# a-ludi/dentist

Measured on AMD Instinct MI355X. Metric: gap-bases closed/sec, higher is better.
Workload: dtype u8

## Files before the change

### dentist_amd/_lib.py

```python
import ctypes
import os
import weakref

import numpy as np

_HERE = os.path.dirname(os.path.abspath(__file__))


def lib_path():
    return os.environ.get("DH_DEV_LIB") or os.path.join(_HERE, "libdentist_hip.so")


class DhError(RuntimeError):
    def __init__(self, code, msg):
        super().__init__(f"libdentist_hip error {code}: {msg}")
        self.code = code


class AlignOpts(ctypes.Structure):
    _fields_ = [(n, ctypes.c_int32) for n in (
        "k", "hmin", "band_shift", "tspace", "min_len", "pen", "xdrop", "max_err_ppm", "max_cand",
        "max_la", "tcap", "strands", "skip_self", "dmax", "width", "kmer_mod", "algo")]


# ... 34 lines not shown
    "contig_left", "status", "nreads", "ref_read", "ref_read_id", "crop_left", "crop_right", "left_aepos",
    "right_abpos", "ins_begin", "ins_end", "comp", "cons_len", "left_diffs", "right_diffs", "join")]
    + [("cons_off", "<i8"), ("contig_right", "<i4"), ("pad", "<i4")])

EXACT_HIT_DTYPE = np.dtype([("query", "<i4"), ("ref", "<i4"), ("begin", "<i8"), ("end", "<i8"), ("complement", "<i4"),
                            ("pad", "<i4")])

LA_DTYPE = np.dtype([("tlen", "<i4"), ("diffs", "<i4"), ("abpos", "<i4"), ("bbpos", "<i4"),
                     ("aepos", "<i4"), ("bepos", "<i4"), ("flags", "<u4"), ("aread", "<i4"),
                     ("bread", "<i4"), ("pad", "<i4"), ("toff", "<i8")])

SYMBOLS = [
    "dh_last_error", "dh_abi_version", "dh_ctx_create", "dh_ctx_destroy", "dh_ctx_sync",
    "dh_default_align_opts", "dh_db_create", "dh_db_destroy", "dh_db_drop_cache", "dh_db_nreads",
    "dh_db_total_bases", "dh_la_set_destroy", "dh_la_set_count", "dh_la_set_trace_len",
    "dh_la_set_records", "dh_la_set_trace", "dh_la_set_tspace", "dh_get_align_stats", "dh_get_cum_stats", "dh_get_mjoin_counts", "dh_get_join_counts", "dh_get_tjoin_counts", "dh_join_hit_capacity",
    "dh_ctx_release_scratch",
    "dh_align_db",
    "dh_las_write", "dh_las_read", "dh_default_process_opts", "dh_collect_spanning", "dh_pileups_destroy",
    "dh_pileups_count", "dh_pileups_get", "dh_process_pileups", "dh_insertions_destroy",
    "dh_insertions_count", "dh_insertions_records", "dh_insertions_bases", "dh_insertions_bases_len",
    "dh_get_process_stats", "dh_dazz_create_dam", "dh_dazz_create_db", "dh_dazz_split", "dh_dazz_open",
    "dh_dazz_close", "dh_dazz_nreads", "dh_dazz_first_id", "dh_dazz_bases", "dh_dazz_offsets",
    "dh_dazz_origin", "dh_dazz_fpulse", "dh_dazz_header", "dh_dazz_read_mask", "dh_dazz_write_mask",
    "dh_db_set_mask", "dh_output_fasta", "dh_tile_qv", "dh_consensus", "dh_las_merge",
    "dh_collect_candidates", "dh_pileups_create", "dh_pileups_select", "dh_align_db_block", "dh_la_set_merge",
    "dh_crop_pileups", "dh_cropped_create", "dh_cropped_destroy", "dh_cropped_npiles", "dh_cropped_records",
    "dh_cropped_nreads", "dh_cropped_pile", "dh_cropped_entry", "dh_cropped_read_id", "dh_cropped_offsets",
    "dh_cropped_bases", "dh_process_cropped", "dh_translate_trace_point", "dh_db_dust", "dh_db_get_mask",
    "dh_dazz_write_track", "dh_dazz_read_track", "dh_dazz_remove", "dh_dazz_flags",
    "dh_pileupdb_write", "dh_pileupdb_read", "dh_insertiondb_write", "dh_insertiondb_read", "dh_insertiondb_merge", "dh_chaindb_destroy",
# ... 312 lines not shown
        _check(lib().dh_get_mjoin_counts(self._h, out, int(reset)))
        return int(out[0]), int(out[1])

    def join_counts(self, reset=False):
        out = (ctypes.c_int64 * 4)()
        lib().dh_get_join_counts.argtypes = [ctypes.c_void_p, ctypes.c_void_p, ctypes.c_int32]
        _check(lib().dh_get_join_counts(self._h, out, int(reset)))
        return tuple(int(x) for x in out)

    def tjoin_counts(self, reset=False):
        out = (ctypes.c_int64 * 4)()
        lib().dh_get_tjoin_counts.argtypes = [ctypes.c_void_p, ctypes.c_void_p, ctypes.c_int32]
        _check(lib().dh_get_tjoin_counts(self._h, out, int(reset)))
        return tuple(int(x) for x in out)

    def cum_stats(self, reset=False):
        st = CumStats()
        _check(lib().dh_get_cum_stats(self._h, ctypes.byref(st), int(reset)))
        return st

    def remap_skipping_reads(self, contigs, reads, contig_ids, read_ids, opts, allowance):
        ci = np.ascontiguousarray(contig_ids, dtype=np.int32)
        ri = np.ascontiguousarray(read_ids, dtype=np.int32)
        h = ctypes.c_void_p()
        L = lib()
        L.dh_remap_skipping_reads.argtypes = [ctypes.c_void_p, ctypes.c_void_p, ctypes.c_void_p, ctypes.c_void_p, ctypes.c_int32,
                                              ctypes.c_void_p, ctypes.c_int32, ctypes.c_void_p, ctypes.c_int32,
                                              ctypes.POINTER(ctypes.c_void_p)]
        _check(L.dh_remap_skipping_reads(self._h, contigs._h, reads._h, ci.ctypes.data, len(ci), ri.ctypes.data, len(ri),
                                         ctypes.byref(opts), int(allowance), ctypes.byref(h)))
# ... 1618 lines not shown
```

### dentist_amd/csrc/dh_align.cpp

```cpp
#include <chrono>
#include <cmath>
#include <cstdio>
#include <cstdlib>
#include <cstring>
#include <numeric>
#include <functional>
#include <memory>
#include <mutex>
#include <thread>

#include "dh_internal.h"
#include "dh_join.h"
#include "dh_mjoin.h"
#include "dh_tjoin.h"
#include "dh_tile.h"
#include "dh_parallel.h"

#define fail dh_fail

#ifdef DH_SEED_PROF
extern "C" void dhk_seed_prof_dump();
extern "C" void dhk_join_prof_dump();
extern "C" void dhk_tile_prof_dump();
#endif
// ... 831 lines not shown
        tj_chunk = true;
    }
    const bool jn = r.use_join || mj_chunk || tj_chunk;
    const JoinView &jvx = mj_chunk ? jv_mj : (tj_chunk ? jv_tj : r.jv);
    const int tier_max = getenv("DH_SEED_NO16K") ? 8192 : 16384;
    const double kmers_per_read = (double)(B->h_off[(size_t)((item0 + ni) >> 1)] - B->h_off[(size_t)(item0 >> 1)]) /
                                  std::max(1, ni / 2) / std::max(1, o.kmer_mod);
    const double mean_hits = tj_chunk ? (double)tj_hits / std::max(1, ni / 2) : kmers_per_read * (2.0 * r.dens + 0.075);
    const bool wave_tier = (mj_chunk || tj_chunk) && ctx->seed_wave_tier && 1.5 * mean_hits <= 512.0 && !getenv("DH_SEED_NO_WAVE_TIER");
    int capj = std::min(std::max(r.cap, 2048), tier_max);
    if (mj_chunk || tj_chunk) {
        capj = 2048;
        while (capj < tier_max && 1.5 * mean_hits > capj) capj *= 2;
        if (wave_tier) capj = 512;
    }
    if (jn && capj > 4096) SCR(SLOT_FSCR, d_fscr, (size_t)ctx->ncu * DH_SEED_FSCR_BLOCKS_PER_CU * (capj > 8192 ? DH_SEED_FSCR_WORDS16 : DH_SEED_FSCR_WORDS))
    if (jn)
        dhk_seed_join(st, capj, r.bv, r.iv, r.dopt, jvx, (int32_t)item0, ni, c.candbase, c.ncandbase, c.nhitsbase, r.d_status,
                      r.d_queue + 1, ctx->ncu, d_fscr, nullptr, 0);
    else
        dhk_seed(st, r.cap, r.bv, r.iv, r.dopt, (int32_t)item0, ni, c.candbase, c.ncandbase, c.nhitsbase, r.d_status,
                 r.d_queue + 1, ctx->ncu, d_fscr);
    HIPCHK(hipGetLastError());
    int32_t status = 0;
    unsigned long long sm[4] = {0, 0, 0, 0};
    dhk_seed_summary(st, r.d_ncand, r.d_nhits, ni, r.d_summary);
    HIPCHK(hipMemcpyAsync(&status, r.d_status, sizeof(int32_t), hipMemcpyDeviceToHost, st));
    HIPCHK(hipMemcpyAsync(sm, r.d_summary, sizeof(sm), hipMemcpyDeviceToHost, st));
    HIPCHK(hipStreamSynchronize(st));
    if (mj_chunk && (status & DH_ST_MJ_POOL) && !(status & DH_ST_MJ_OVERFLOW) && !getenv("DH_MJOIN_PAGES")) {
        unsigned long long cnt2[2] = {0, 0};
        HIPCHK(hipMemcpyAsync(cnt2, r.d_mjctr_last + 10, sizeof(cnt2), hipMemcpyDeviceToHost, st));
        status &= ~DH_ST_MJ_POOL;
        HIPCHK(hipMemcpyAsync(r.d_status, &status, sizeof(int32_t), hipMemcpyHostToDevice, st));
// ... 36 lines not shown
            fprintf(stderr, "[seeds] %zu of %d reads overflow the wavefront-per-read tier: not used by this context any more\n", big.size(), ni / 2);
    }
    size_t redo_all = (size_t)ni / 50 + 8;
    if (r.cap >= 8192) redo_all = (size_t)ni / 4;
    if (const char *e = getenv("DH_SEED_BIG_PCT")) redo_all = (size_t)((double)ni * atof(e) / 200.0);
    if (getenv("DH_TRACE") && !big.empty())
        fprintf(stderr, "[seeds] cap %d: %zu of %d reads overflow (whole chunk again above %zu)\n", r.cap, big.size(), ni / 2, redo_all);
    if (!jn && big.size() > redo_all && r.cap < 16384) {
        r.cap *= 2;
        *redo = true;
        return DH_OK;
    }
    if (mj_chunk) ctx->mj_chunks++;
    if (tj_chunk) ctx->tj_last_hits += (int64_t)tj_hits;
    r.mj_skip_chunk = false;
    if (jn && capj < tier_max && !big.empty()) {
        std::vector<int32_t> huge;
        int32_t gcap2 = 0;
        for (int tier = capj < 2048 ? 2048 : 8192; tier <= tier_max; tier = tier < 8192 ? 8192 : tier * 2) {
            if (tier <= capj) continue;
            std::vector<int32_t> mid;
            huge.clear();
            gcap2 = 0;
            for (int32_t rd : big) {
                const size_t it = (size_t)(2 * (int64_t)rd - item0);
                const int32_t nh = r.h_nhits[it] + r.h_nhits[it + 1];
                if (nh <= tier)
                    mid.push_back(rd);
                else {
                    huge.push_back(rd);
                    gcap2 = std::max(gcap2, nh);
                }
            }
            if (!mid.empty()) {
                int32_t *d_mid;
                uint64_t *d_fscr2;
                SCR(SLOT_MID_LIST, d_mid, mid.size())
                SCR(SLOT_FSCR, d_fscr2, (size_t)ctx->ncu * DH_SEED_FSCR_BLOCKS_PER_CU * (tier > 8192 ? DH_SEED_FSCR_WORDS16 : DH_SEED_FSCR_WORDS))
                HIPCHK(hipMemcpyAsync(d_mid, mid.data(), sizeof(int32_t) * mid.size(), hipMemcpyHostToDevice, st));
                HIPCHK(hipMemsetAsync(r.d_queue + 1, 0, sizeof(uint32_t), st));
                dhk_seed_join(st, tier, r.bv, r.iv, r.dopt, jvx, (int32_t)item0, ni, c.candbase, c.ncandbase, c.nhitsbase, r.d_status,
                              r.d_queue + 1, ctx->ncu, d_fscr2, d_mid, (int32_t)mid.size());
                HIPCHK(hipGetLastError());
                HIPCHK(hipStreamSynchronize(st));
            }
            if (getenv("DH_TRACE"))
                fprintf(stderr, "[seeds] join tiers: %zu reads redone with %d entries, %zu left\n", mid.size(), tier, huge.size());
            big = huge;
        }
        gcap = gcap2;
    }
    if (!big.empty()) {
        if (gcap > (1 << 22)) return fail(DH_EOVERFLOW, "seed filter: more than 4M k-mer hits for one sequence; lower -t");
        int32_t pow2 = 1;
        while (pow2 < gcap) pow2 <<= 1;
        const size_t slab_words = 2 * (size_t)pow2 + ((size_t)pow2 + 1) / 2;
        const size_t per_launch = std::max<size_t>(1, (size_t)(2ull << 30) / (slab_words * 8));
// ... 495 lines not shown
```

### dentist_amd/csrc/dh_api.cpp

```cpp
#include <cstring>

#include "dh_internal.h"

static_assert(sizeof(dh_align_opts) == sizeof(DhOpts), "opts layout");
static_assert(sizeof(dh_la) == sizeof(DhLa), "la layout");
static_assert(sizeof(dh_la) == 48, "la size");

static thread_local std::string g_err;

int dh_fail(int code, const std::string &msg)
{
    g_err = msg;
    return code;
}
#define fail dh_fail

extern "C" const char *dh_last_error(void) { return g_err.c_str(); }
extern "C" int32_t dh_abi_version(void) { return 4; }



extern "C" int dh_ctx_create(int32_t device, void *stream, dh_ctx **out)
{
    if (!out) return fail(DH_EINVAL, "dh_ctx_create: out is NULL");
// ... 115 lines not shown
    if (reset) c->mj_chunks = c->mj_fallbacks = 0;
    return DH_OK;
}

extern "C" int dh_get_tjoin_counts(dh_ctx *c, int64_t *out4, int32_t reset)
{
    if (!c || !out4) return fail(DH_EINVAL, "dh_get_tjoin_counts: NULL");
    out4[0] = c->tj_calls;
    out4[1] = c->tj_fallbacks;
    out4[2] = c->tj_last_hits;
    out4[3] = c->tj_reruns;
    if (reset) c->tj_calls = c->tj_fallbacks = c->tj_last_hits = c->tj_reruns = 0;
    return DH_OK;
}

extern "C" int dh_get_join_counts(dh_ctx *c, int64_t *out4, int32_t reset)
{
    if (!c || !out4) return fail(DH_EINVAL, "dh_get_join_counts: NULL");
    out4[0] = c->join_launches;
    out4[1] = c->join_reruns;
    out4[2] = c->join_last_hits;
    out4[3] = c->join_first_cap;
    if (reset) c->join_launches = c->join_reruns = c->join_last_hits = c->join_first_cap = 0;
    return DH_OK;
}

extern "C" int dh_get_align_stats(dh_ctx *c, dh_align_stats *out)
{
    if (!c || !out) return fail(DH_EINVAL, "dh_get_align_stats: NULL");
    *out = c->stats;
// ... 32 lines not shown
```

### dentist_amd/csrc/dh_batch.cpp

```cpp
#include <atomic>
#include <cstdlib>
#include <cstring>
#include <exception>
#include <string>
#include <thread>

#include "dh_process.h"
#include "dh_parallel.h"

using namespace dhp;

extern "C" {
void dhk_gather_ranges16(hipStream_t st, const uint16_t *src, const int64_t *desc, int32_t n, uint16_t *dst);
}

namespace {

int select_trace_ranges(const dh_db *reads, const dh_la_set *set, const dh_pileups *piles, std::vector<int64_t> &desc, int64_t &total)
{
    const int64_t n = (int64_t)set->la.size();
    std::vector<uint8_t> need((size_t)reads->n, 0);
    for (const auto &t : piles->triples)
        for (size_t x = 0; x + 2 < t.size(); x += 3) {
            if (t[x] < 0 || t[x] >= reads->n) return dh_fail(DH_EINVAL, "dh_process_pileups_set: read id out of range");
// ... 200 lines not shown
        a.ms_index += b.ms_index; a.ms_seed += b.ms_seed; a.ms_wave += b.ms_wave; a.ms_gather += b.ms_gather;
        a.wave_launches += b.wave_launches; a.wave_cells += b.wave_cells; a.alignments += b.alignments; a.las += b.las;
        a.aligned_bp += b.aligned_bp; a.trace_values += b.trace_values; a.hits += b.hits; a.b_bases += b.b_bases;
        b = dh_cum_stats();
        dh_ctx *sc = ctx->sub[k - 1];
        ctx->join_launches += sc->join_launches;
        ctx->join_reruns += sc->join_reruns;
        ctx->join_last_hits += sc->join_last_hits;
        ctx->join_first_cap += sc->join_first_cap;
        sc->join_launches = sc->join_reruns = sc->join_last_hits = sc->join_first_cap = 0;
        ctx->tj_calls += sc->tj_calls;
        ctx->tj_fallbacks += sc->tj_fallbacks;
        ctx->tj_last_hits += sc->tj_last_hits;
        ctx->tj_reruns += sc->tj_reruns;
        sc->tj_calls = sc->tj_fallbacks = sc->tj_last_hits = sc->tj_reruns = 0;
    }
}

void fold_part_stats(const std::vector<PartOut> &po)
{
    ProcStats &ps = dh_proc_stats();
    for (size_t k = 1; k < po.size(); k++) {
        for (int i = 0; i < 7; i++) ps.ms[i] = std::max(ps.ms[i], po[k].st.ms[i]);
        for (int i = 0; i < 3; i++) ps.counters[i] += po[k].st.counters[i];
        for (int i = 0; i < 4; i++) ps.work[i] += po[k].st.work[i];
    }
}

dh_insertions *append_insertions(std::vector<PartOut> &po)
{
// ... 56 lines not shown
```

### dentist_amd/csrc/dh_internal.h

```cpp
#ifndef DH_INTERNAL_H
#define DH_INTERNAL_H

#include "../../include/dentist_hip.h"

#include <hip/hip_runtime.h>

#include <algorithm>
#include <string>
#include <new>
#include <utility>
#include <vector>

#include "dh_device.h"

#define DB_PAD 64
#define PK_PAD 128

hipError_t dh_dev_alloc(void **p, size_t bytes);
void dh_dev_free(void *p);
void dh_dev_trim();
template <typename T>
inline hipError_t dh_dev_alloc(T **p, size_t bytes)
{
    return dh_dev_alloc((void **)p, bytes);
// ... 79 lines not shown

#define DH_TJ_HIT_RATE0 0.14

struct dh_ctx {
    int device = 0;
    hipStream_t stream = nullptr;
    bool own_stream = false;
    int ncu = 0;
    hipEvent_t ev[8] = {};
    hipStream_t cstream = nullptr;
    hipEvent_t cev[4] = {};
    dh_align_stats stats = {};
    dh_cum_stats cum = {};
    double mj_hit_frac = 0.2;
    int seed_wave_tier = 1;
    int64_t mj_chunks = 0, mj_fallbacks = 0;
    int64_t tj_calls = 0, tj_fallbacks = 0, tj_last_hits = 0, tj_reruns = 0;
    double tj_hit_rate = DH_TJ_HIT_RATE0;
    double join_hit_rate = DH_JOIN_HIT_RATE0;
    int64_t join_launches = 0, join_reruns = 0, join_last_hits = 0, join_first_cap = 0;
    int32_t near_best_ppm = -1;
    dh_ctx *sub[3] = {nullptr, nullptr, nullptr};
    struct Arena {
        void *p = nullptr;
        size_t cap = 0;
    } arena[DH_SLOT_COUNT];
};
int dh_scratch(dh_ctx *ctx, DhSlot id, size_t bytes, void **out);
int dh_db_set_pflags(struct dh_db *db, const uint8_t *flags);

// ... 180 lines not shown
```

### dentist_amd/csrc/dh_join.h

```cpp
#ifndef DH_JOIN_H
#define DH_JOIN_H
#include <stdint.h>

#include "dh_device.h"

#define JP_THREADS 512
#define JP_PER 16
#define JP_POS (JP_THREADS * JP_PER)
#define JOIN_MAX_READS 512
#define JOIN_MAX_LEN (1 << 21)
#define JOIN_MAX_SLICES 512
#define JOIN_CAP 4096
#define JOIN_FILL 2300
#define JOIN_THREADS 512

#define DH_ST_JOIN_OVERFLOW 0x8
#define DH_ST_JOIN_HITCAP 0x10

struct JoinView {
    const int32_t *gfirst;
    const int32_t *gns;
    const int32_t *pfirst;
    const int2 *pblk;
    const int64_t *psubrow;
// ... 6 lines not shown
    unsigned long long *cursor;
    int64_t hits_cap;
    int32_t *status;
    int32_t npart, njoin;
    int32_t ns_fixed, read0;
};

#ifdef __cplusplus
extern "C" {
#endif
void dhk_join_part(hipStream_t st, JoinView jv, DbView B, int32_t k, int32_t kmer_mod);
void dhk_join(hipStream_t st, JoinView jv, DbView B, DhOpts o, const int64_t *goff, int32_t sepv);
void dhk_join_hist(hipStream_t st, JoinView jv, const int32_t *group, int32_t nreads, unsigned int *out4);
void dhk_seed_join(hipStream_t st, int cap, DbView B, IndexView ix, DhOpts o, JoinView jv, int32_t item0, int32_t nitems,
                   DhCand *cand, int32_t *ncand, int32_t *nhits, int32_t *status, uint32_t *queue, int32_t ncu,
                   uint64_t *fscr, const int32_t *read_list, int32_t nlist);
void dhk_seed_big_join(hipStream_t st, DbView B, IndexView ix, DhOpts o, JoinView jv, const int32_t *read_list,
                       int32_t nreads, uint64_t *gbuf, int32_t gcap, DhCand *cand, int32_t *ncand, int32_t *nhits,
                       int32_t *status, uint32_t *queue, int32_t ncu);
#ifdef __cplusplus
}
#endif
#endif
```

### dentist_amd/csrc/dh_seed.hip

```cpp
#include <hip/hip_runtime.h>
#include <type_traits>
#include <algorithm>
#include <cstdlib>
#include <stdio.h>
#include <stdint.h>
#include <stdlib.h>

#include "dh_device.h"
#include "dh_join.h"

#define LANES 64

#include "dh_kmer.h"


__device__ int g_seed_sort_refine = 1;
#define HIT_QBITS 24
#define HIT_QMASK ((1u << HIT_QBITS) - 1u)
#define SEED_THREADS 512
#define SEED_LOOKUP_THREADS 512
#define SEED_CCAP 256

__device__ __forceinline__ int64_t hitD(uint64_t h) { return (int64_t)(h >> HIT_QBITS); }
__device__ __forceinline__ int32_t hitQ(uint64_t h) { return (int32_t)(h & HIT_QMASK); }

__device__ __forceinline__ int32_t hit_cov(const uint64_t *h, int32_t i, int32_t k)
{
    if (i > 0 && hitD(h[i - 1]) == hitD(h[i])) {
        const int32_t dq = hitQ(h[i]) - hitQ(h[i - 1]);
        return dq < k ? dq : k;
    }
    return k;
}

#ifdef DH_SEED_PROF
__device__ unsigned long long g_seed_prof[12];
#define SP(i) if (tid == 0) { const unsigned long long t_ = wall_clock64(); atomicAdd(&g_seed_prof[i], t_ - tp_); tp_ = t_; }
#else
#define SP(i)
#endif
#define HIT_DBITS 39
template <int LCAP, bool JOIN, int NT, int CC>
__device__ void seed_item(const DbView &B, const IndexView &ix, const JoinView &jv,
                          const DhOpts &o, int32_t read0, int32_t work, int32_t slab,
                          DhCand *__restrict__ cand_out, int32_t *__restrict__ ncand_out,
                          int32_t *__restrict__ nhits_out, int32_t *__restrict__ status,
                          uint64_t *__restrict__ gbuf, int32_t gcap, const int32_t *__restrict__ read_list)
{
    __shared__ uint64_t lhits[LCAP > 0 ? LCAP : 1];
    __shared__ DhCand cands[2 * CC];
    __shared__ int64_t cband[2 * CC];
    __shared__ int32_t s_n, s_nc;

    const int32_t r = read_list ? read_list[work] : read0 + work;
    const int32_t item = 2 * r;
    uint64_t *hits = LCAP > 0 ? lhits : gbuf + (int64_t)slab * (2 * (int64_t)gcap + (gcap + 1) / 2);
    const int32_t CAP = LCAP > 0 ? LCAP : gcap;
    const int tid = threadIdx.x;
#ifdef DH_SEED_PROF
    unsigned long long tp_ = wall_clock64();
#endif
    if (tid == 0) {
        s_n = 0;
        s_nc = 0;
    }
    __syncthreads();
    const int64_t bo = B.off[r];
    const int32_t blen = (int32_t)(B.off[r + 1] - bo);
    const uint8_t *b = B.bases + bo;
    const uint64_t grp = B.group ? (uint64_t)B.group[r] : 0ull;
    const int k = o.k;
    const uint64_t mask = (1ull << (2 * k)) - 1;
    const int32_t npos = blen - k + 1;
    constexpr uint64_t ORI = 1ull << 63, PAL = 1ull << 62;

    if (JOIN) {
        uint64_t *segb = (uint64_t *)cands;
        uint32_t *sego = (uint32_t *)(cands + CC) + 1;
        __shared__ uint32_t s_jw[NT / LANES];
        const int32_t ns = jv.gns ? jv.gns[B.group[r]] : jv.ns_fixed;
        const int64_t srow = jv.gns ? jv.segrow[r] : (int64_t)(r - jv.read0) * jv.ns_fixed;
        uint32_t c = 0;
        if (tid < ns) {
            const uint64_t sg = jv.segtab[srow + tid];
            c = (uint32_t)(sg & 0xFFFFFFull);
            segb[tid] = sg >> 24;
        }
        uint32_t incl = c;
        for (int off = 1; off < LANES; off <<= 1) {
            const uint32_t up = __shfl_up(incl, off, LANES);
            if ((tid & (LANES - 1)) >= off) incl += up;
        }
        if ((tid & (LANES - 1)) == LANES - 1) s_jw[tid / LANES] = incl;
// ... 182 lines not shown
    if (n > CAP) {
        if (tid == 0) {
            if (LCAP == 0) atomicOr(status, DH_ST_HIT_OVERFLOW);
            ncand_out[item] = ncand_out[item + 1] = LCAP > 0 ? -1 : 0;
            nhits_out[item] = n;
            nhits_out[item + 1] = 0;
        }
        return;
    }
    if (n == 0) {
        if (tid == 0) ncand_out[item] = ncand_out[item + 1] = nhits_out[item] = nhits_out[item + 1] = 0;
        return;
    }
    int32_t N = 1;
    while (N < n) N <<= 1;
    constexpr bool SMALL = NT < SEED_THREADS;
    if (SMALL) {
        constexpr int E8 = LCAP / NT > 0 ? LCAP / NT : 1;
        uint64_t ky[E8];
        int32_t rk8[E8];
#pragma unroll
        for (int u = 0; u < E8; u++) {
            const int32_t i = tid + u * NT;
            ky[u] = i < n ? hits[i] : ~0ull;
            rk8[u] = 0;
        }
#define DH_RANK_KEYS(M_)                                                   \
    for (int32_t x = 0; x < n; x++) {                                      \
        const uint64_t h = hits[x];                                        \
        _Pragma("unroll") for (int u = 0; u < (M_ < E8 ? M_ : E8); u++) rk8[u] += h < ky[u] ? 1 : 0; \
    }
        if (n <= 2 * NT) {
// ... 15 lines not shown
        if (tid < n) {
            key = hits[tid];
#pragma unroll 4
            for (int32_t x = 0; x < n; x++) rk += hits[x] < key ? 1 : 0;
        }
        __syncthreads();
        if (tid < n)
            hits[rk] = key;
        else if (tid < N)
            hits[tid] = ~0ull;
        N = 1;
    } else if (LCAP == 0 || ((LCAP <= 8192 || JOIN) && (JOIN || LCAP >= 4096))) {
        constexpr int E = LCAP >= NT ? LCAP / NT : 1;
        constexpr int NB = 2048, NBH = NB / 2, SORT_BMAX = LCAP == 0 ? 384 : 256;
        constexpr uint64_t DM = (1ull << HIT_DBITS) - 1;
        static_assert(SMALL || sizeof(cands) >= NB * sizeof(uint32_t), "bucket counters overlay the candidate array");
        uint32_t *bcnt = (uint32_t *)cands;
        __shared__ unsigned long long s_dmin, s_dmax;
        __shared__ uint32_t s_bw[NT / LANES];
        __shared__ uint32_t s_bmax;
        constexpr int HV = 8, NB2 = 1024;
        constexpr bool REFINE = LCAP > 0 && !SMALL;
        static_assert(!REFINE || sizeof(cband) >= NB2 * sizeof(uint32_t), "the second pass's counters overlay the band array");
        uint32_t *fcnt = (uint32_t *)cband;
        __shared__ uint32_t s_nheavy, s_heavy[HV];
        for (int32_t i = tid; i < NB; i += NT) bcnt[i] = 0;
        if (tid == 0) {
            s_dmin = ~0ull;
            s_dmax = 0ull;
            s_bmax = 0;
            s_nheavy = 0;
        }
        unsigned long long dmin = ~0ull, dmax = 0ull;
        for (int32_t i = tid; i < n; i += NT) {
            const unsigned long long d = (hits[i] >> HIT_QBITS) & DM;
            dmin = d < dmin ? d : dmin;
            dmax = d > dmax ? d : dmax;
        }
        for (int off = LANES / 2; off > 0; off >>= 1) {
// ... 222 lines not shown
                    if (REFINE)
                        for (uint32_t hv = 0; hv < nheavy; hv++) heavy = heavy || s_heavy[hv] == bk;
                    if (heavy)
                        dst[u] = (uint32_t)i;
                    else
                        dst[u] = b0 + count_below(b0, b1, key, sh <= 32 - HIT_QBITS);
                }
            }
            __syncthreads();
#pragma unroll
            for (int u = 0; u < E; u++)
                if (tid + u * NT < n) hits[dst[u]] = ke[u];
            N = 1;
        } else {
#ifdef DH_SEED_PROF
            if (tid == 0) atomicAdd(&g_seed_prof[10], 1ull);
#endif
            for (int32_t i = n + tid; i < N; i += NT) hits[i] = ~0ull;
        }
    } else {
        for (int32_t i = n + tid; i < N; i += NT) hits[i] = ~0ull;
    }
    __syncthreads();
    for (int32_t kk = 2; kk <= N; kk <<= 1) {
        for (int32_t j = kk >> 1; j > 0; j >>= 1) {
            const bool cross = j >= 128;
            if (cross) __syncthreads();
            constexpr int SORT_U = (LCAP == 0 || LCAP >= 4096) ? 8 : 4;
            for (int32_t p0 = tid; p0 < (N >> 1); p0 += NT * SORT_U) {
                uint64_t xs[SORT_U], ys[SORT_U];
#pragma unroll
// ... 27 lines not shown
    __syncthreads();
    if (tid == 0) {
        int32_t lo = 0, hi = n;
        while (lo < hi) {
            const int32_t mid = (lo + hi) >> 1;
            if (hits[mid] >> 63)
                hi = mid;
            else
                lo = mid + 1;
        }
        nhits_out[item] = lo;
        nhits_out[item + 1] = n - lo;
    }
    SP(1)
    constexpr bool FASTB = LCAP <= 8192 || (JOIN && LCAP == 16384);
    constexpr bool FB_LDS = LCAP > 0 && LCAP <= 4096;
    constexpr bool FB_BIG = LCAP == 0;
    constexpr bool FB_WIDE = LCAP == 0 || LCAP == 16384;
    using bsum_t = typename std::conditional<FB_WIDE, uint64_t, uint32_t>::type;
    using bhead_t = typename std::conditional<FB_WIDE, uint32_t, uint16_t>::type;
    constexpr int HSH = FB_WIDE ? 32 : 18;
    constexpr bsum_t CMASK = ((bsum_t)1 << HSH) - 1;
    __shared__ uint32_t bsum_l[FB_LDS ? LCAP : 1];
    __shared__ uint16_t bhead_l[FB_LDS ? LCAP : 1];
    bsum_t *bsum = FB_LDS ? (bsum_t *)bsum_l
                          : (FB_BIG ? (bsum_t *)(hits + gcap) : (bsum_t *)(gbuf + (int64_t)slab * gcap));
    bhead_t *bhead = FB_LDS ? (bhead_t *)bhead_l : (bhead_t *)(bsum + (LCAP > 0 ? LCAP : gcap));
    __shared__ bsum_t s_wsum[NT / LANES];
    __shared__ int32_t s_nbig;
    constexpr int NBIG = NT < SEED_THREADS ? 8 : ((LCAP > 0 && LCAP <= 4096) ? 128 : 64);
    __shared__ int32_t bigc[NBIG][4];
    __shared__ unsigned long long s_bestkeys[NBIG];
    const int bs = o.band_shift;
    auto emit_cand = [&](int32_t slot, int32_t best_first, int32_t P, int64_t band) {
        const int64_t D = hitD(hits[best_first]) & ((1ll << HIT_DBITS) - 1);
        const int32_t q = hitQ(hits[best_first]);
        const int64_t gv = D - ix.sepv + q;
        const int32_t lo = ix.page_seq[gv >> 12];
        cands[slot].score = P;
        cands[slot].aseq = lo;
        cands[slot].apos = (int32_t)(gv - ix.goff[lo]);
        cands[slot].bpos = q;
        cband[slot] = band;
    };
    auto serial_seed = [&](int32_t i, int32_t e1) {
// ... 70 lines not shown
            if (slot >= 2 * CC) continue;
            if (e1 - i > 16) {
                const int32_t bslot = atomicAdd(&s_nbig, 1);
                if (bslot < NBIG) {
                    bigc[bslot][0] = i;
                    bigc[bslot][1] = e1;
                    bigc[bslot][2] = P;
                    bigc[bslot][3] = slot;
                    continue;
                }
            }
            emit_cand(slot, serial_seed(i, e1), P, band);
        }
        __syncthreads();
        SP(8)
        constexpr int GW = 16;
        const int32_t nbig = min(s_nbig, NBIG);
        const int gl = tid & (GW - 1);
        for (int32_t bc = tid / GW; bc < nbig; bc += NT / GW) {
            const int32_t i = bigc[bc][0], e1 = bigc[bc][1];
            unsigned long long best = 0ull;
            int32_t carry = i;
            for (int32_t base = i; base < e1; base += GW) {
                const int32_t x = base + gl;
                const bool valid = x < e1;
                const uint64_t h = valid ? hits[x] : 0ull;
                const uint64_t hp = valid && x > i ? hits[x - 1] : 0ull;
                const uint64_t hn = x + 1 < e1 ? hits[x + 1] : 0ull;
                const bool linked = valid && x > i && hitD(h) == hitD(hp) && (hitQ(h) - hitQ(hp)) <= k;
                int32_t f = valid && !linked ? x : -1;
                for (int off = 1; off < GW; off <<= 1) {
// ... 30 lines not shown
            for (; j < n && (hitD(hits[j]) >> bs) == band; j++) cov0 += hit_cov(hits, j, k);
            for (; j < n && (hitD(hits[j]) >> bs) == band + 1; j++) cov1 += hit_cov(hits, j, k);
            e1 = j;
            for (; j < n && (hitD(hits[j]) >> bs) == band + 2; j++) cov2 += hit_cov(hits, j, k);
            const int32_t P = cov0 + cov1, Pm1 = covm1 + cov0, Pp1 = cov1 + cov2;
            if (P < o.hmin || P < Pm1 || P <= Pp1) continue;
            const int32_t slot = atomicAdd(&s_nc, 1);
            if (slot < 2 * CC) emit_cand(slot, serial_seed(i, e1), P, band);
        }
    }
    __syncthreads();
    SP(3)
    int32_t nc = s_nc;
    if (nc > 2 * CC) {
        if (tid == 0) {
            ncand_out[item] = ncand_out[item + 1] = NT < SEED_THREADS ? -1 : -2;
            if (NT < SEED_THREADS) {
                nhits_out[item] = n;
                nhits_out[item + 1] = 0;
            }
        }
        return;
    }
    __shared__ int32_t crank_s[LCAP > 0 ? 1 : 2 * CC];
    int32_t *crank = LCAP > 0 ? (int32_t *)lhits : crank_s;
    __shared__ int32_t s_ncs[2];
    constexpr int BSTR = HIT_DBITS;
    auto strand_of = [&](int32_t c) { return (int32_t)((cband[c] >> (BSTR - bs)) & 1); };
    if (tid < 2) s_ncs[tid] = 0;
    __syncthreads();
    for (int32_t c = tid; c < nc; c += NT) {
        const int32_t st = strand_of(c);
// ... 16 lines not shown
        int32_t pos = rank;
        if (o.skip_self == 2) {
            pos = 0;
            const int32_t ac = cands[c].aseq;
#pragma unroll 4
            for (int32_t x = 0; x < nc; x++) {
                const int32_t ax = cands[x].aseq, rx = crank[x];
                pos += (strand_of(x) == st && rx < o.max_cand && (ax < ac || (ax == ac && rx < rank))) ? 1 : 0;
            }
        }
        cand_out[(int64_t)(item + st) * o.max_cand + pos] = cands[c];
    }
    if (tid < 2) ncand_out[item + tid] = s_ncs[tid] < o.max_cand ? s_ncs[tid] : o.max_cand;
    SP(4)
#ifdef DH_SEED_PROF
    if (tid == 0) atomicAdd(&g_seed_prof[7], 1ull);
#endif
}
template <int LCAP, bool JOIN, int NT = SEED_THREADS, int CC = SEED_CCAP>
__global__ void __launch_bounds__(NT, NT < SEED_THREADS ? 4 : ((LCAP > 0 && LCAP <= 2048) ? 6 : (LCAP == 16384 ? 2 : 4)))
k_seed(DbView B, IndexView ix, JoinView jv, DhOpts o, int32_t read0,
       int32_t nreads, DhCand *__restrict__ cand_out, int32_t *__restrict__ ncand_out,
       int32_t *__restrict__ nhits_out, int32_t *__restrict__ status, uint64_t *__restrict__ gbuf,
       int32_t gcap, const int32_t *__restrict__ read_list, uint32_t *__restrict__ queue)
{
    __shared__ int32_t s_work;
    constexpr int32_t BATCH = (JOIN && LCAP > 0 && LCAP <= 2048) ? 8 : 1;
    for (;;) {
        __syncthreads();
        if (threadIdx.x == 0) s_work = (int32_t)atomicAdd(queue, (uint32_t)BATCH);
        __syncthreads();
        const int32_t work0 = s_work;
        if (work0 >= nreads) break;
#pragma unroll 1
        for (int32_t wi = 0; wi < BATCH; wi++) {
            const int32_t work = work0 + wi;
            if (work >= nreads) break;
            if (wi) __syncthreads();
            seed_item<LCAP, JOIN, NT, CC>(B, ix, jv, o, read0, work, (int32_t)blockIdx.x, cand_out, ncand_out, nhits_out,
                                          status, gbuf, gcap, read_list);
        }
    }
}
#define SEED_INST(C, J)                                                                           \
    template __global__ void k_seed<C, J>(DbView, IndexView, JoinView, DhOpts, int32_t, int32_t,  \
                                          DhCand *, int32_t *, int32_t *, int32_t *, uint64_t *, int32_t, \
                                          const int32_t *, uint32_t *);
SEED_INST(1024, false)
SEED_INST(2048, false)
SEED_INST(4096, false)
SEED_INST(8192, false)
SEED_INST(16384, false)
SEED_INST(0, false)
SEED_INST(2048, true)
template __global__ void k_seed<512, true, 64, 32>(DbView, IndexView, JoinView, DhOpts, int32_t, int32_t, DhCand *, int32_t *, int32_t *,
                                                   int32_t *, uint64_t *, int32_t, const int32_t *, uint32_t *);
SEED_INST(4096, true)
SEED_INST(8192, true)
SEED_INST(16384, true)
SEED_INST(0, true)


template <int C, bool J, int NT, int CC>
static int seed_grid(int32_t nitems, int32_t ncu)
{
    static int per_cu = 0;
    if (per_cu == 0) {
        int nb = 0;
        if (hipOccupancyMaxActiveBlocksPerMultiprocessor(&nb, k_seed<C, J, NT, CC>, NT, 0) != hipSuccess || nb < 1)
            nb = 1;
        per_cu = nb;
    }
    int use = per_cu;
    if (const char *e = getenv("DH_SEED_BLOCKS_PER_CU")) use = std::max(1, std::min(per_cu, atoi(e)));
    const int64_t g = (int64_t)use * ncu;
    return (int)(g < nitems ? g : nitems);
}

struct SeedLaunch {
    hipStream_t st;
    DbView B;
    IndexView ix;
    JoinView jv;
    DhOpts o;
    int32_t read0, nreads;
    DhCand *cand;
// ... 38 lines not shown
    else
        launch_seed<16384, false>(a, nullptr, 0);
}

extern "C" void dhk_seed_big(hipStream_t st, DbView B, IndexView ix, DhOpts o,
                             const int32_t *read_list, int32_t nreads, uint64_t *gbuf, int32_t gcap, DhCand *cand,
                             int32_t *ncand, int32_t *nhits, int32_t *status, uint32_t *queue, int32_t ncu)
{
    if (nreads <= 0) return;
    const SeedLaunch a = {st, B, ix, JoinView{}, o, 0, nreads, cand, ncand, nhits, status, read_list, queue, ncu};
    launch_seed<0, false>(a, gbuf, gcap);
}

extern "C" void dhk_seed_join(hipStream_t st, int cap, DbView B, IndexView ix, DhOpts o, JoinView jv, int32_t item0,
                              int32_t nitems, DhCand *cand, int32_t *ncand, int32_t *nhits, int32_t *status,
                              uint32_t *queue, int32_t ncu, uint64_t *fscr, const int32_t *read_list, int32_t nlist)
{
    if (nitems <= 0 || (read_list && nlist <= 0)) return;
    seed_sort_switch();
    const SeedLaunch a = {st,     B,     ix,     jv,        o,     item0 / 2, read_list ? nlist : nitems / 2, cand, ncand,
                          nhits,  status, read_list, queue, ncu};
    if (cap <= 512)
        launch_seed<512, true, 64, 32>(a, nullptr, 0);
    else if (cap <= 2048)
        launch_seed<2048, true>(a, nullptr, 0);
    else if (cap <= 4096)
        launch_seed<4096, true>(a, nullptr, 0);
    else if (cap <= 8192)
        launch_seed<8192, true>(a, fscr, DH_SEED_FSCR_WORDS);
    else
        launch_seed<16384, true>(a, fscr, DH_SEED_FSCR_WORDS16);
}

extern "C" void dhk_seed_big_join(hipStream_t st, DbView B, IndexView ix, DhOpts o, JoinView jv, const int32_t *read_list,
                                  int32_t nreads, uint64_t *gbuf, int32_t gcap, DhCand *cand, int32_t *ncand,
                                  int32_t *nhits, int32_t *status, uint32_t *queue, int32_t ncu)
{
    if (nreads <= 0) return;
    const SeedLaunch a = {st, B, ix, jv, o, 0, nreads, cand, ncand, nhits, status, read_list, queue, ncu};
    launch_seed<0, true>(a, gbuf, gcap);
}

#ifdef DH_SEED_PROF
extern "C" void dhk_seed_prof_dump()
{
    unsigned long long h[12];
    (void)hipMemcpyFromSymbol(h, HIP_SYMBOL(g_seed_prof), sizeof(h));
    fprintf(stderr, "[seed prof] blocks %llu: lookup %.1f sort %.1f bcov %.1f bands %.1f rank %.1f us/block (of the sort: buckets %.1f scatter %.1f; of the bands: heads %.1f long ranges %.1f; %llu reads through the network)\n", h[7], h[0] / 100.0 / h[7], h[1] / 100.0 / h[7], h[2] / 100.0 / h[7], h[3] / 100.0 / h[7], h[4] / 100.0 / h[7], h[5] / 100.0 / h[7], h[6] / 100.0 / h[7], h[8] / 100.0 / h[7], h[9] / 100.0 / h[7], h[10]);
    unsigned long long z[12] = {0};
    (void)hipMemcpyToSymbol(HIP_SYMBOL(g_seed_prof), z, sizeof(z));
}
#endif

extern "C" __global__ void __launch_bounds__(256)
k_seed_summary(const int32_t *__restrict__ ncand, const int32_t *__restrict__ nhits, int32_t n, unsigned long long *__restrict__ out)
{
    unsigned long long h = 0, c = 0, big = 0, gave = 0;
    for (int32_t i = blockIdx.x * blockDim.x + threadIdx.x; i < n; i += gridDim.x * blockDim.x) {
        const int32_t nc = ncand[i];
        h += (unsigned long long)max(nhits[i], 0);
        c += (unsigned long long)max(nc, 0);
        big += nc == -1 ? 1ull : 0ull;
        gave += nc == -2 ? 1ull : 0ull;
// ... 28 lines not shown
```

### include/dentist_hip.h

```cpp
#ifndef DENTIST_HIP_H
#define DENTIST_HIP_H

#include <stddef.h>
#include <stdint.h>

#ifdef __cplusplus
extern "C" {
#endif

#define DH_OK 0
#define DH_EINVAL (-1)
#define DH_ENODEV (-2)
#define DH_EHIP (-3)
#define DH_EOVERFLOW (-4)
#define DH_EIO (-5)
#define DH_ENOMEM (-6)

const char *dh_last_error(void);
int32_t dh_abi_version(void);

typedef struct dh_ctx dh_ctx;
int dh_ctx_create(int32_t device, void *stream, dh_ctx **out);
void dh_ctx_destroy(dh_ctx *ctx);
int dh_ctx_sync(dh_ctx *ctx);
// ... 58 lines not shown
    int32_t wave_launches;
    int32_t overflow_items;
    int64_t big_items;
} dh_align_stats;
int dh_get_align_stats(dh_ctx *ctx, dh_align_stats *out);

typedef struct {
    double ms_index, ms_seed, ms_wave, ms_gather;
    int64_t wave_launches, wave_cells, alignments, las, aligned_bp, trace_values, hits, b_bases;
} dh_cum_stats;
int dh_get_cum_stats(dh_ctx *ctx, dh_cum_stats *out, int32_t reset);
int dh_ctx_release_scratch(dh_ctx *ctx);
int dh_get_mjoin_counts(dh_ctx *ctx, int64_t *out2, int32_t reset);
int dh_get_join_counts(dh_ctx *ctx, int64_t *out4, int32_t reset);
int dh_get_tjoin_counts(dh_ctx *ctx, int64_t *out4, int32_t reset);
int64_t dh_join_hit_capacity(const int64_t *bases, const int32_t *reads, int32_t ngroups, int32_t skip_self, double rate,
                             int64_t free_bytes);

int dh_align_db(dh_ctx *ctx, dh_db *A, dh_db *B, const dh_align_opts *opts, int32_t select_best,
                dh_la_set **out);
void dh_set_near_best(int32_t ppm);
int dh_ctx_set_near_best(dh_ctx *ctx, int32_t ppm);

int dh_align_db_block(dh_ctx *ctx, dh_db *A, dh_db *B, int32_t first, int32_t count,
                      const dh_align_opts *opts, int32_t select_best, dh_la_set **out);
int dh_align_db_transposed(dh_ctx *ctx, dh_db *A, dh_db *B, const dh_align_opts *opts, int32_t want_best,
                           dh_la_set **out, dh_la_set **out_transposed);
int dh_la_set_merge(const dh_la_set *const *sets, int32_t nsets, dh_la_set **out);

int dh_las_write(const char *path, const dh_la *las, int64_t n, const uint16_t *trace,
// ... 470 lines not shown
```

Before: 2.438 million.

## Add a 256-thread middle seed tier for 2048-hit join chunks

Adds a new k_seed<2048, true, 256, 64> instantiation used for join chunks whose expected hits fit 2048. It overlays segment tables and bucket counters on the band-sum LDS arrays to shrink shared memory, and uses a smaller candidate cap, aiming at more resident blocks per CU and less per-read waste. Reads that overflow are redone by the existing 512-thread tiers, and the context turns the tier off if more than a quarter overflow. Profiling counters move to per-block LDS accumulation, and a tier-count API is added.

Result: faster. 2.518 million, median of 6 (+3.3%).

```diff
diff --git a/dentist_amd/_lib.py b/dentist_amd/_lib.py
--- a/dentist_amd/_lib.py
+++ b/dentist_amd/_lib.py
@@ -72,7 +72,7 @@
     "dh_last_error", "dh_abi_version", "dh_ctx_create", "dh_ctx_destroy", "dh_ctx_sync",
     "dh_default_align_opts", "dh_db_create", "dh_db_destroy", "dh_db_drop_cache", "dh_db_nreads",
     "dh_db_total_bases", "dh_la_set_destroy", "dh_la_set_count", "dh_la_set_trace_len",
-    "dh_la_set_records", "dh_la_set_trace", "dh_la_set_tspace", "dh_get_align_stats", "dh_get_cum_stats", "dh_get_mjoin_counts", "dh_get_join_counts", "dh_get_tjoin_counts", "dh_join_hit_capacity",
+    "dh_la_set_records", "dh_la_set_trace", "dh_la_set_tspace", "dh_get_align_stats", "dh_get_cum_stats", "dh_get_mjoin_counts", "dh_get_join_counts", "dh_get_tjoin_counts", "dh_get_seed_tier_counts", "dh_join_hit_capacity",
     "dh_ctx_release_scratch",
     "dh_align_db",
     "dh_las_write", "dh_las_read", "dh_default_process_opts", "dh_collect_spanning", "dh_pileups_destroy",
@@ -415,6 +415,12 @@
         _check(lib().dh_get_tjoin_counts(self._h, out, int(reset)))
         return tuple(int(x) for x in out)
 
+    def seed_tier_counts(self, reset=False):
+        out = (ctypes.c_int64 * 2)()
+        lib().dh_get_seed_tier_counts.argtypes = [ctypes.c_void_p, ctypes.c_void_p, ctypes.c_int32]
+        _check(lib().dh_get_seed_tier_counts(self._h, out, int(reset)))
+        return int(out[0]), int(out[1])
+
     def cum_stats(self, reset=False):
         st = CumStats()
         _check(lib().dh_get_cum_stats(self._h, ctypes.byref(st), int(reset)))
diff --git a/dentist_amd/csrc/dh_align.cpp b/dentist_amd/csrc/dh_align.cpp
--- a/dentist_amd/csrc/dh_align.cpp
+++ b/dentist_amd/csrc/dh_align.cpp
@@ -869,10 +869,12 @@
         while (capj < tier_max && 1.5 * mean_hits > capj) capj *= 2;
         if (wave_tier) capj = 512;
     }
+    const bool mid_tier = (mj_chunk || tj_chunk) && !wave_tier && capj == 2048 && ctx->seed_mid_tier &&
+                          (!mj_chunk || c.mv.nseg <= 256) && !getenv("DH_SEED_NO_MID_TIER");
     if (jn && capj > 4096) SCR(SLOT_FSCR, d_fscr, (size_t)ctx->ncu * DH_SEED_FSCR_BLOCKS_PER_CU * (capj > 8192 ? DH_SEED_FSCR_WORDS16 : DH_SEED_FSCR_WORDS))
     if (jn)
         dhk_seed_join(st, capj, r.bv, r.iv, r.dopt, jvx, (int32_t)item0, ni, c.candbase, c.ncandbase, c.nhitsbase, r.d_status,
-                      r.d_queue + 1, ctx->ncu, d_fscr, nullptr, 0);
+                      r.d_queue + 1, ctx->ncu, d_fscr, nullptr, 0, mid_tier ? 1 : 0);
     else
         dhk_seed(st, r.cap, r.bv, r.iv, r.dopt, (int32_t)item0, ni, c.candbase, c.ncandbase, c.nhitsbase, r.d_status,
                  r.d_queue + 1, ctx->ncu, d_fscr);
@@ -939,11 +941,20 @@
     if (mj_chunk) ctx->mj_chunks++;
     if (tj_chunk) ctx->tj_last_hits += (int64_t)tj_hits;
     r.mj_skip_chunk = false;
-    if (jn && capj < tier_max && !big.empty()) {
+    if (mid_tier) {
+        ctx->seed_mid_chunks++;
+        ctx->seed_mid_redone += (int64_t)big.size();
+        if (big.size() * 4 > (size_t)(ni / 2)) ctx->seed_mid_tier = 0;
+        if (getenv("DH_TRACE"))
+            fprintf(stderr, "[seeds] middle tier (256 threads, 2048 hits, 64 band pairs): %d reads, %zu redone by the 512-thread tiers%s\n",
+                    ni / 2, big.size(), ctx->seed_mid_tier ? "" : ": not used by this context any more");
+    }
+    const int held = mid_tier ? 0 : capj;
+    if (jn && held < tier_max && !big.empty()) {
         std::vector<int32_t> huge;
         int32_t gcap2 = 0;
-        for (int tier = capj < 2048 ? 2048 : 8192; tier <= tier_max; tier = tier < 8192 ? 8192 : tier * 2) {
-            if (tier <= capj) continue;
+        for (int tier = held < 2048 ? 2048 : 8192; tier <= tier_max; tier = tier < 8192 ? 8192 : tier * 2) {
+            if (tier <= held) continue;
             std::vector<int32_t> mid;
             huge.clear();
             gcap2 = 0;
@@ -965,7 +976,7 @@
                 HIPCHK(hipMemcpyAsync(d_mid, mid.data(), sizeof(int32_t) * mid.size(), hipMemcpyHostToDevice, st));
                 HIPCHK(hipMemsetAsync(r.d_queue + 1, 0, sizeof(uint32_t), st));
                 dhk_seed_join(st, tier, r.bv, r.iv, r.dopt, jvx, (int32_t)item0, ni, c.candbase, c.ncandbase, c.nhitsbase, r.d_status,
-                              r.d_queue + 1, ctx->ncu, d_fscr2, d_mid, (int32_t)mid.size());
+                              r.d_queue + 1, ctx->ncu, d_fscr2, d_mid, (int32_t)mid.size(), 0);
                 HIPCHK(hipGetLastError());
                 HIPCHK(hipStreamSynchronize(st));
             }
diff --git a/dentist_amd/csrc/dh_api.cpp b/dentist_amd/csrc/dh_api.cpp
--- a/dentist_amd/csrc/dh_api.cpp
+++ b/dentist_amd/csrc/dh_api.cpp
@@ -153,6 +153,15 @@
     return DH_OK;
 }
 
+extern "C" int dh_get_seed_tier_counts(dh_ctx *c, int64_t *out2, int32_t reset)
+{
+    if (!c || !out2) return fail(DH_EINVAL, "dh_get_seed_tier_counts: NULL");
+    out2[0] = c->seed_mid_chunks;
+    out2[1] = c->seed_mid_redone;
+    if (reset) c->seed_mid_chunks = c->seed_mid_redone = 0;
+    return DH_OK;
+}
+
 extern "C" int dh_get_join_counts(dh_ctx *c, int64_t *out4, int32_t reset)
 {
     if (!c || !out4) return fail(DH_EINVAL, "dh_get_join_counts: NULL");
diff --git a/dentist_amd/csrc/dh_batch.cpp b/dentist_amd/csrc/dh_batch.cpp
--- a/dentist_amd/csrc/dh_batch.cpp
+++ b/dentist_amd/csrc/dh_batch.cpp
@@ -238,6 +238,9 @@
         ctx->tj_last_hits += sc->tj_last_hits;
         ctx->tj_reruns += sc->tj_reruns;
         sc->tj_calls = sc->tj_fallbacks = sc->tj_last_hits = sc->tj_reruns = 0;
+        ctx->seed_mid_chunks += sc->seed_mid_chunks;
+        ctx->seed_mid_redone += sc->seed_mid_redone;
+        sc->seed_mid_chunks = sc->seed_mid_redone = 0;
     }
 }
 
diff --git a/dentist_amd/csrc/dh_internal.h b/dentist_amd/csrc/dh_internal.h
--- a/dentist_amd/csrc/dh_internal.h
+++ b/dentist_amd/csrc/dh_internal.h
@@ -117,6 +117,8 @@
     dh_cum_stats cum = {};
     double mj_hit_frac = 0.2;
     int seed_wave_tier = 1;
+    int seed_mid_tier = 1;
+    int64_t seed_mid_chunks = 0, seed_mid_redone = 0;
     int64_t mj_chunks = 0, mj_fallbacks = 0;
     int64_t tj_calls = 0, tj_fallbacks = 0, tj_last_hits = 0, tj_reruns = 0;
     double tj_hit_rate = DH_TJ_HIT_RATE0;
diff --git a/dentist_amd/csrc/dh_join.h b/dentist_amd/csrc/dh_join.h
--- a/dentist_amd/csrc/dh_join.h
+++ b/dentist_amd/csrc/dh_join.h
@@ -44,7 +44,7 @@
 void dhk_join_hist(hipStream_t st, JoinView jv, const int32_t *group, int32_t nreads, unsigned int *out4);
 void dhk_seed_join(hipStream_t st, int cap, DbView B, IndexView ix, DhOpts o, JoinView jv, int32_t item0, int32_t nitems,
                    DhCand *cand, int32_t *ncand, int32_t *nhits, int32_t *status, uint32_t *queue, int32_t ncu,
-                   uint64_t *fscr, const int32_t *read_list, int32_t nlist);
+                   uint64_t *fscr, const int32_t *read_list, int32_t nlist, int32_t mid_tier);
 void dhk_seed_big_join(hipStream_t st, DbView B, IndexView ix, DhOpts o, JoinView jv, const int32_t *read_list,
                        int32_t nreads, uint64_t *gbuf, int32_t gcap, DhCand *cand, int32_t *ncand, int32_t *nhits,
                        int32_t *status, uint32_t *queue, int32_t ncu);
diff --git a/dentist_amd/csrc/dh_seed.hip b/dentist_amd/csrc/dh_seed.hip
--- a/dentist_amd/csrc/dh_seed.hip
+++ b/dentist_amd/csrc/dh_seed.hip
@@ -35,7 +35,12 @@
 
 #ifdef DH_SEED_PROF
 __device__ unsigned long long g_seed_prof[12];
-#define SP(i) if (tid == 0) { const unsigned long long t_ = wall_clock64(); atomicAdd(&g_seed_prof[i], t_ - tp_); tp_ = t_; }
+__device__ __forceinline__ unsigned long long *seed_prof_lds()
+{
+    __shared__ unsigned long long s_prof[12];
+    return s_prof;
+}
+#define SP(i) if (tid == 0) { const unsigned long long t_ = wall_clock64(); seed_prof_lds()[i] += t_ - tp_; tp_ = t_; }
 #else
 #define SP(i)
 #endif
@@ -47,9 +52,14 @@
                           int32_t *__restrict__ nhits_out, int32_t *__restrict__ status,
                           uint64_t *__restrict__ gbuf, int32_t gcap, const int32_t *__restrict__ read_list)
 {
+    constexpr bool RANK_ALL = LCAP > 0 && NT <= LANES && LCAP <= 8 * NT;
+    constexpr bool SLIM = LCAP > 0 && LCAP <= 4096 && NT > LANES && NT < SEED_THREADS;
+    constexpr bool FB_LDS = LCAP > 0 && LCAP <= 4096;
     __shared__ uint64_t lhits[LCAP > 0 ? LCAP : 1];
     __shared__ DhCand cands[2 * CC];
     __shared__ int64_t cband[2 * CC];
+    __shared__ __attribute__((aligned(8))) uint32_t bsum_l[FB_LDS ? LCAP : 1];
+    __shared__ __attribute__((aligned(8))) uint16_t bhead_l[FB_LDS ? LCAP : 1];
     __shared__ int32_t s_n, s_nc;
 
     const int32_t r = read_list ? read_list[work] : read0 + work;
@@ -75,8 +85,12 @@
     constexpr uint64_t ORI = 1ull << 63, PAL = 1ull << 62;
 
     if (JOIN) {
-        uint64_t *segb = (uint64_t *)cands;
-        uint32_t *sego = (uint32_t *)(cands + CC) + 1;
+        static_assert(SLIM || (sizeof(cands) / 2 >= NT * sizeof(uint64_t) && sizeof(cands) / 2 >= (NT + 1) * sizeof(uint32_t)),
+                      "segment tables overlay the candidate array");
+        static_assert(!SLIM || (sizeof(bsum_l) >= NT * sizeof(uint64_t) && sizeof(bhead_l) >= (NT + 1) * sizeof(uint32_t)),
+                      "segment tables overlay the band arrays");
+        uint64_t *segb = SLIM ? (uint64_t *)bsum_l : (uint64_t *)cands;
+        uint32_t *sego = (SLIM ? (uint32_t *)bhead_l : (uint32_t *)(cands + CC)) + 1;
         __shared__ uint32_t s_jw[NT / LANES];
         const int32_t ns = jv.gns ? jv.gns[B.group[r]] : jv.ns_fixed;
         const int64_t srow = jv.gns ? jv.segrow[r] : (int64_t)(r - jv.read0) * jv.ns_fixed;
@@ -289,8 +303,7 @@
     }
     int32_t N = 1;
     while (N < n) N <<= 1;
-    constexpr bool SMALL = NT < SEED_THREADS;
-    if (SMALL) {
+    if (RANK_ALL) {
         constexpr int E8 = LCAP / NT > 0 ? LCAP / NT : 1;
         uint64_t ky[E8];
         int32_t rk8[E8];
@@ -336,15 +349,19 @@
         constexpr int E = LCAP >= NT ? LCAP / NT : 1;
         constexpr int NB = 2048, NBH = NB / 2, SORT_BMAX = LCAP == 0 ? 384 : 256;
         constexpr uint64_t DM = (1ull << HIT_DBITS) - 1;
-        static_assert(SMALL || sizeof(cands) >= NB * sizeof(uint32_t), "bucket counters overlay the candidate array");
-        uint32_t *bcnt = (uint32_t *)cands;
+        static_assert(NB % NT == 0 && NT % LANES == 0, "every thread scans NB / NT counters, whole wavefronts");
+        static_assert(RANK_ALL || SLIM || sizeof(cands) >= NB * sizeof(uint32_t), "bucket counters overlay the candidate array");
+        static_assert(!SLIM || sizeof(bsum_l) >= NB * sizeof(uint32_t), "bucket counters overlay the prefix sums");
+        uint32_t *bcnt = SLIM ? (uint32_t *)bsum_l : (uint32_t *)cands;
         __shared__ unsigned long long s_dmin, s_dmax;
         __shared__ uint32_t s_bw[NT / LANES];
         __shared__ uint32_t s_bmax;
         constexpr int HV = 8, NB2 = 1024;
-        constexpr bool REFINE = LCAP > 0 && !SMALL;
-        static_assert(!REFINE || sizeof(cband) >= NB2 * sizeof(uint32_t), "the second pass's counters overlay the band array");
-        uint32_t *fcnt = (uint32_t *)cband;
+        constexpr bool REFINE = LCAP > 0 && !RANK_ALL;
+        static_assert(!REFINE || SLIM || sizeof(cband) >= NB2 * sizeof(uint32_t), "the second pass's counters overlay the band array");
+        static_assert(!SLIM || sizeof(bhead_l) >= NB2 * sizeof(uint32_t), "the second pass's counters overlay the band heads");
+        static_assert(NB2 % NT == 0 && (LCAP == 0 || LCAP % NT == 0 || LCAP < NT), "NB2 / NT counters, LCAP / NT hits per thread");
+        uint32_t *fcnt = SLIM ? (uint32_t *)bhead_l : (uint32_t *)cband;
         __shared__ uint32_t s_nheavy, s_heavy[HV];
         for (int32_t i = tid; i < NB; i += NT) bcnt[i] = 0;
         if (tid == 0) {
@@ -597,7 +614,7 @@
             N = 1;
         } else {
 #ifdef DH_SEED_PROF
-            if (tid == 0) atomicAdd(&g_seed_prof[10], 1ull);
+            if (tid == 0) seed_prof_lds()[10] += 1ull;
 #endif
             for (int32_t i = n + tid; i < N; i += NT) hits[i] = ~0ull;
         }
@@ -655,21 +672,18 @@
     }
     SP(1)
     constexpr bool FASTB = LCAP <= 8192 || (JOIN && LCAP == 16384);
-    constexpr bool FB_LDS = LCAP > 0 && LCAP <= 4096;
     constexpr bool FB_BIG = LCAP == 0;
     constexpr bool FB_WIDE = LCAP == 0 || LCAP == 16384;
     using bsum_t = typename std::conditional<FB_WIDE, uint64_t, uint32_t>::type;
     using bhead_t = typename std::conditional<FB_WIDE, uint32_t, uint16_t>::type;
     constexpr int HSH = FB_WIDE ? 32 : 18;
     constexpr bsum_t CMASK = ((bsum_t)1 << HSH) - 1;
-    __shared__ uint32_t bsum_l[FB_LDS ? LCAP : 1];
-    __shared__ uint16_t bhead_l[FB_LDS ? LCAP : 1];
     bsum_t *bsum = FB_LDS ? (bsum_t *)bsum_l
                           : (FB_BIG ? (bsum_t *)(hits + gcap) : (bsum_t *)(gbuf + (int64_t)slab * gcap));
     bhead_t *bhead = FB_LDS ? (bhead_t *)bhead_l : (bhead_t *)(bsum + (LCAP > 0 ? LCAP : gcap));
     __shared__ bsum_t s_wsum[NT / LANES];
     __shared__ int32_t s_nbig;
-    constexpr int NBIG = NT < SEED_THREADS ? 8 : ((LCAP > 0 && LCAP <= 4096) ? 128 : 64);
+    constexpr int NBIG = NT <= LANES ? 8 : (SLIM ? 16 : ((LCAP > 0 && LCAP <= 4096) ? 128 : 64));
     __shared__ int32_t bigc[NBIG][4];
     __shared__ unsigned long long s_bestkeys[NBIG];
     const int bs = o.band_shift;
@@ -770,7 +784,7 @@
         }
         __syncthreads();
         SP(8)
-        constexpr int GW = 16;
+        constexpr int GW = SLIM ? LANES : 16;
         const int32_t nbig = min(s_nbig, NBIG);
         const int gl = tid & (GW - 1);
         for (int32_t bc = tid / GW; bc < nbig; bc += NT / GW) {
@@ -831,8 +845,8 @@
     int32_t nc = s_nc;
     if (nc > 2 * CC) {
         if (tid == 0) {
-            ncand_out[item] = ncand_out[item + 1] = NT < SEED_THREADS ? -1 : -2;
-            if (NT < SEED_THREADS) {
+            ncand_out[item] = ncand_out[item + 1] = CC < SEED_CCAP ? -1 : -2;
+            if (CC < SEED_CCAP) {
                 nhits_out[item] = n;
                 nhits_out[item + 1] = 0;
             }
@@ -879,11 +893,11 @@
     if (tid < 2) ncand_out[item + tid] = s_ncs[tid] < o.max_cand ? s_ncs[tid] : o.max_cand;
     SP(4)
 #ifdef DH_SEED_PROF
-    if (tid == 0) atomicAdd(&g_seed_prof[7], 1ull);
+    if (tid == 0) seed_prof_lds()[7] += 1ull;
 #endif
 }
 template <int LCAP, bool JOIN, int NT = SEED_THREADS, int CC = SEED_CCAP>
-__global__ void __launch_bounds__(NT, NT < SEED_THREADS ? 4 : ((LCAP > 0 && LCAP <= 2048) ? 6 : (LCAP == 16384 ? 2 : 4)))
+__global__ void __launch_bounds__(NT, NT <= LANES ? 4 : (NT < SEED_THREADS ? 5 : ((LCAP > 0 && LCAP <= 2048) ? 6 : (LCAP == 16384 ? 2 : 4))))
 k_seed(DbView B, IndexView ix, JoinView jv, DhOpts o, int32_t read0,
        int32_t nreads, DhCand *__restrict__ cand_out, int32_t *__restrict__ ncand_out,
        int32_t *__restrict__ nhits_out, int32_t *__restrict__ status, uint64_t *__restrict__ gbuf,
@@ -891,6 +905,10 @@
 {
     __shared__ int32_t s_work;
     constexpr int32_t BATCH = (JOIN && LCAP > 0 && LCAP <= 2048) ? 8 : 1;
+#ifdef DH_SEED_PROF
+    if (threadIdx.x == 0)
+        for (int i = 0; i < 12; i++) seed_prof_lds()[i] = 0;
+#endif
     for (;;) {
         __syncthreads();
         if (threadIdx.x == 0) s_work = (int32_t)atomicAdd(queue, (uint32_t)BATCH);
@@ -906,6 +924,11 @@
                                           status, gbuf, gcap, read_list);
         }
     }
+#ifdef DH_SEED_PROF
+    if (threadIdx.x == 0)
+        for (int i = 0; i < 12; i++)
+            if (seed_prof_lds()[i]) atomicAdd(&g_seed_prof[i], seed_prof_lds()[i]);
+#endif
 }
 #define SEED_INST(C, J)                                                                           \
     template __global__ void k_seed<C, J>(DbView, IndexView, JoinView, DhOpts, int32_t, int32_t,  \
@@ -920,6 +943,8 @@
 SEED_INST(2048, true)
 template __global__ void k_seed<512, true, 64, 32>(DbView, IndexView, JoinView, DhOpts, int32_t, int32_t, DhCand *, int32_t *, int32_t *,
                                                    int32_t *, uint64_t *, int32_t, const int32_t *, uint32_t *);
+template __global__ void k_seed<2048, true, 256, 64>(DbView, IndexView, JoinView, DhOpts, int32_t, int32_t, DhCand *, int32_t *, int32_t *,
+                                                     int32_t *, uint64_t *, int32_t, const int32_t *, uint32_t *);
 SEED_INST(4096, true)
 SEED_INST(8192, true)
 SEED_INST(16384, true)
@@ -935,6 +960,8 @@
         if (hipOccupancyMaxActiveBlocksPerMultiprocessor(&nb, k_seed<C, J, NT, CC>, NT, 0) != hipSuccess || nb < 1)
             nb = 1;
         per_cu = nb;
+        if (getenv("DH_TRACE"))
+            fprintf(stderr, "[seeds] k_seed<%d, %s, %d, %d>: %d resident blocks per CU\n", C, J ? "true" : "false", NT, CC, nb);
     }
     int use = per_cu;
     if (const char *e = getenv("DH_SEED_BLOCKS_PER_CU")) use = std::max(1, std::min(per_cu, atoi(e)));
@@ -1003,7 +1030,8 @@
 
 extern "C" void dhk_seed_join(hipStream_t st, int cap, DbView B, IndexView ix, DhOpts o, JoinView jv, int32_t item0,
                               int32_t nitems, DhCand *cand, int32_t *ncand, int32_t *nhits, int32_t *status,
-                              uint32_t *queue, int32_t ncu, uint64_t *fscr, const int32_t *read_list, int32_t nlist)
+                              uint32_t *queue, int32_t ncu, uint64_t *fscr, const int32_t *read_list, int32_t nlist,
+                              int32_t mid_tier)
 {
     if (nitems <= 0 || (read_list && nlist <= 0)) return;
     seed_sort_switch();
@@ -1011,6 +1039,8 @@
                           nhits,  status, read_list, queue, ncu};
     if (cap <= 512)
         launch_seed<512, true, 64, 32>(a, nullptr, 0);
+    else if (cap <= 2048 && mid_tier)
+        launch_seed<2048, true, 256, 64>(a, nullptr, 0);
     else if (cap <= 2048)
         launch_seed<2048, true>(a, nullptr, 0);
     else if (cap <= 4096)
@@ -1035,7 +1065,10 @@
 {
     unsigned long long h[12];
     (void)hipMemcpyFromSymbol(h, HIP_SYMBOL(g_seed_prof), sizeof(h));
-    fprintf(stderr, "[seed prof] blocks %llu: lookup %.1f sort %.1f bcov %.1f bands %.1f rank %.1f us/block (of the sort: buckets %.1f scatter %.1f; of the bands: heads %.1f long ranges %.1f; %llu reads through the network)\n", h[7], h[0] / 100.0 / h[7], h[1] / 100.0 / h[7], h[2] / 100.0 / h[7], h[3] / 100.0 / h[7], h[4] / 100.0 / h[7], h[5] / 100.0 / h[7], h[6] / 100.0 / h[7], h[8] / 100.0 / h[7], h[9] / 100.0 / h[7], h[10]);
+    const double per = h[7] ? 1.0 / 100.0 / (double)h[7] : 0.0;
+    fprintf(stderr, "[seed prof] reads %llu: fill %.1f sort %.1f (buckets %.1f scatter %.1f ranks %.1f) bcov %.1f bands %.1f (heads %.1f long ranges %.1f emit %.1f) rank %.1f us/read; %llu reads through the network\n",
+            h[7], h[0] * per, (h[5] + h[6] + h[1]) * per, h[5] * per, h[6] * per, h[1] * per, h[2] * per, (h[8] + h[9] + h[3]) * per,
+            h[8] * per, h[9] * per, h[3] * per, h[4] * per, h[10]);
     unsigned long long z[12] = {0};
     (void)hipMemcpyToSymbol(HIP_SYMBOL(g_seed_prof), z, sizeof(z));
 }
diff --git a/include/dentist_hip.h b/include/dentist_hip.h
--- a/include/dentist_hip.h
+++ b/include/dentist_hip.h
@@ -96,6 +96,7 @@
 int dh_get_mjoin_counts(dh_ctx *ctx, int64_t *out2, int32_t reset);
 int dh_get_join_counts(dh_ctx *ctx, int64_t *out4, int32_t reset);
 int dh_get_tjoin_counts(dh_ctx *ctx, int64_t *out4, int32_t reset);
+int dh_get_seed_tier_counts(dh_ctx *ctx, int64_t *out2, int32_t reset);
 int64_t dh_join_hit_capacity(const int64_t *bases, const int32_t *reads, int32_t ngroups, int32_t skip_self, double rate,
                              int64_t free_bytes);
 
```
